# sarahappleby/VAMP

Measured on AMD Instinct MI355X. Metric: walker-steps/sec (log-posterior evals/sec), higher is better.
Workload: dtype f64

## Files before the change

### vamp_amd/csrc/vamp_hip.hip

```cpp
#include <hip/hip_runtime.h>
#include <dlfcn.h>

#include <algorithm>
#include <atomic>
#include <chrono>
#include <cmath>
#include <cstdint>
#include <cstdio>
#include <cstdlib>
#include <cstring>
#include <new>
#include <string>
#include <vector>

#include "../../include/vamp_hip.h"
#include "abi_state.hpp"
#include "draws.hpp"
#include "host_plan.hpp"
#include "map_search.hpp"
#include "voigt_math.hpp"
#include "ff_predicates.hpp"
#include "ff_moments.hpp"

#ifndef VAMP_EARLY_LOADS
#define VAMP_EARLY_LOADS 1
#endif
#ifndef VAMP_BLEND_PASS_LINES
#define VAMP_BLEND_PASS_LINES 4
#endif
#ifndef VAMP_MID_MIN_K
#define VAMP_MID_MIN_K 3
#endif
#ifndef VAMP_MID_MIN_P
#define VAMP_MID_MIN_P 96
#endif
#ifndef VAMP_X_PREFETCH
#define VAMP_X_PREFETCH 0
#endif

#ifndef VAMP_MIN_WAVES
#define VAMP_MIN_WAVES 3
#endif
#ifndef VAMP_EARLY_LNP
#define VAMP_EARLY_LNP 1
#endif
#ifndef VAMP_SR_EARLY
#define VAMP_SR_EARLY 0
#endif
#ifndef VAMP_XCD_MAP
#define VAMP_XCD_MAP 0
#endif
#ifndef VAMP_WIDE_NODES
#define VAMP_WIDE_NODES 1
#endif
#ifndef VAMP_LPT
#define VAMP_LPT 1
#endif
#ifndef VAMP_FLUX_EXP_DROP
#define VAMP_FLUX_EXP_DROP 2
#endif
#ifndef VAMP_FF_R2_M4
#define VAMP_FF_R2_M4 100.0
#define VAMP_FF_R2_M3 300.0
#define VAMP_FF_R2_M2 2000.0
#endif
#ifndef VAMP_F32_FAR_CORE
#define VAMP_F32_FAR_CORE 1
#endif
#ifndef VAMP_CORE_FASTPATH
#define VAMP_CORE_FASTPATH 1
#endif
#ifndef VAMP_MID_NODES
#define VAMP_MID_NODES 1
#endif
#ifndef VAMP_MID_Z2
#define VAMP_MID_Z2 30.25
#endif
#ifndef VAMP_WIDE_MAX
#define VAMP_WIDE_MAX 0.75
#endif
#ifndef VAMP_F32_LEAN_STAGE
#define VAMP_F32_LEAN_STAGE 1
#endif
#ifndef VAMP_TILE_MOMENTS
#define VAMP_TILE_MOMENTS 2
#endif
#ifndef VAMP_NODE_PASS
#define VAMP_NODE_PASS 1
#endif
#ifndef VAMP_NP_CLASS_RUNS
#define VAMP_NP_CLASS_RUNS 1
#endif
#ifndef VAMP_DEAL_ADJ
#define VAMP_DEAL_ADJ 1
#endif
#ifndef VAMP_SUPER_NODES
#define VAMP_SUPER_NODES 0
#endif
#ifndef VAMP_TAB_PAIR
#define VAMP_TAB_PAIR 0
#endif
#ifndef VAMP_TILE_HEAD
#define VAMP_TILE_HEAD 0
#endif
namespace {

constexpr int KMAX = 16;
constexpr int KMAX_ALL = VAMP_MAX_COMPONENTS;
static_assert(KMAX_ALL >= KMAX && KMAX_ALL < 64, "lane k stages line k; one spare lane for sd");
constexpr int WAVES_PER_BLOCK = 4;
constexpr long long PACK_MIN_WALKERS = 16384;
constexpr int RES_MAX_MOVERS = 128;
#ifndef VAMP_RES_WAVES
#define VAMP_RES_WAVES 8
#endif
constexpr int RES_MAX_WAVES = VAMP_RES_WAVES;
constexpr int BLOCK = 64 * WAVES_PER_BLOCK;
constexpr int DMAX = 4 * KMAX_ALL + 1;
#ifndef VAMP_SPLIT_MAX_WALKERS
#define VAMP_SPLIT_MAX_WALKERS (1ll << 62)
#endif
constexpr long long SPLIT_MAX_WALKERS = VAMP_SPLIT_MAX_WALKERS;

constexpr double C_LIGHT = 2.98e8;
constexpr double SIGMA0 = 0.0263;
constexpr double SQRT_LN2 = 0.83255461115769775635;
constexpr double SQRT_PI = 1.77245385090551602730;
constexpr double FWHM_PER_SIGMA = 2.35482004503094938202;
constexpr double NEG_INF = -__builtin_huge_val();

using vamp::RegionDev;

struct LineRec {
    double c;
    double s;
    double y;
    double amp;
    double pole;
    double hy;
    double xcap;
    double w8, w25;
    double wmid;
};

#ifndef VAMP_PARTS
#define VAMP_PARTS 4
#endif
constexpr int PARTS = VAMP_PARTS;
template <int KCAP, bool OWN_DTAB> struct WalkerLds;
#ifdef VAMP_STAMPS
__device__ unsigned long long g_stamps[2 * 8192];
__device__ unsigned int g_stamp_n;
#define VAMP_STAMP(tag)                                                                          \
    do {                                                                                         \
        if (blockIdx.x == 0 && threadIdx.x == 0) {                                               \
            const unsigned int n_ = g_stamp_n;                                                   \
            if (n_ < 8192) { g_stamps[2 * n_] = (tag); g_stamps[2 * n_ + 1] = __builtin_amdgcn_s_memtime(); g_stamp_n = n_ + 1; } \
        }                                                                                        \
    } while (0)
#define VAMP_STAMP_AFTER(tag, v) do { asm volatile("" :: "v"(v)); VAMP_STAMP(tag); } while (0)
#else
#define VAMP_STAMP(tag) do {} while (0)
#define VAMP_STAMP_AFTER(tag, v) do {} while (0)
#endif
#ifndef VAMP_SPLIT_WAVES
#define VAMP_SPLIT_WAVES 4
#endif
#ifndef VAMP_SPLIT_WAVES_F32
#define VAMP_SPLIT_WAVES_F32 4
#endif
#ifndef VAMP_F32_TABLES
#define VAMP_F32_TABLES 1
#endif
template <int LPW_, int KCAP_, bool TAIL_, int WPB_, bool SPLIT_ = false, bool TABS_ = SPLIT_, bool FF_ = (LPW_ == 64)>
struct Pack {
    static constexpr int LPW = LPW_, KCAP = KCAP_, SUBS = 64 / LPW_;
    static constexpr bool TAIL = TAIL_;
    static constexpr bool SPLIT = SPLIT_;
    static constexpr bool TABS = TABS_;
    static constexpr bool FF = FF_;
// ... 833 lines not shown
            const LineRec ln = L.line[k];
            double X[T], H[T];
#pragma unroll
            for (int t = 0; t < T; ++t) X[t] = fabs(xi[t] - ln.c) * ln.s;
            if (TAB && (((unsigned)zonemasks >> k) & 1u)) {
                table_eval_tile<T>(tab + k * vamp::TAB_LINE, X, H);
            } else {
                tile_voigt<T, TAB>(ln, dtab_row<PK>(L, k), X, H, TAB ? tab + k * vamp::TAB_LINE : nullptr, dct + FF_EXP);
            }
#pragma unroll
            for (int t = 0; t < T; ++t) tau[t] = fma(ln.amp, H[t], tau[t]);
        }
#endif
        double fi[T], wi[T];
        if (nfar + nwide > 0) {
            double u[T];
#pragma unroll
            for (int t = 0; t < T; ++t) u[t] = ut[base + 64 * t + lane];
#ifndef VAMP_SKIP_FFNODES
            double fs_wide = 0.0;
            if constexpr (WIDE) {
                if (nwide > 0) {
                    fs_wide = ff_wide_nodes<typename PK::Lds>(L, Sx.widelist[j], dct, tab, lane, nwide, mid, half);
                }
            }
            ff_coefficients<typename PK::Lds, GUARD>(L, Sx, Sx.farlist[j], dct, lane, nfar, mid, half, fs_wide);
#endif
#if VAMP_EARLY_LOADS
#pragma unroll
            for (int t = 0; t < T; ++t) {
                fi[t] = f[base + 64 * t + lane];
                wi[t] = wt[base + 64 * t + lane];
            }
            __builtin_amdgcn_sched_barrier(0);
#endif
#ifndef VAMP_SKIP_CLENSHAW
            ff_horner<double, T>(Sx, u, up, tau);
#endif
        } else {
#if VAMP_EARLY_LOADS
#pragma unroll
            for (int t = 0; t < T; ++t) {
                fi[t] = f[base + 64 * t + lane];
                wi[t] = wt[base + 64 * t + lane];
            }
            __builtin_amdgcn_sched_barrier(0);
#endif
        }
        int eoff = FF_EXP;
        asm volatile("" : "+s"(eoff));
        const double* ec = dct + eoff;
#pragma unroll
        for (int t = 0; t < T; ++t) {
#if !VAMP_EARLY_LOADS
            fi[t] = f[base + 64 * t + lane];
            wi[t] = wt[base + 64 * t + lane];
#endif
#ifdef VAMP_SKIP_EXP
            const double m = 1.0 - tau[t];
#else
            const double m = vamp::exp_taylor_tab<VAMP_FLUX_EXP_DROP>(-tau[t], ec);
#endif
            const double r = (fi[t] - m) * wi[t];
            chi = fma(r, r, chi);
        }
    }
    }
}

#if VAMP_NODE_PASS && VAMP_TILE_MOMENTS != 1 && !VAMP_X_PREFETCH && !defined(VAMP_SKIP_NEAR) && !defined(VAMP_SKIP_FFNODES) && \
    !defined(VAMP_SKIP_CLENSHAW) && !defined(VAMP_SKIP_EXP)
#define VAMP_NODE_PASS_ON 1
#else
#define VAMP_NODE_PASS_ON 0
#endif
#if VAMP_NODE_PASS_ON
__device__ __forceinline__ unsigned ff_fold16(unsigned long long m) {
    const unsigned h = (unsigned)m | (unsigned)(m >> 32);
    return (h | (h >> 16)) & 0xffffu;
}
#if VAMP_SUPER_NODES && VAMP_DEAL_ADJ
#define VAMP_SUPER_ON 1
#include "ff_super.inc"
struct NodeSets { unsigned far, n6, n4, n3, wide, dist, d3; double Mid, Half; };
#else
#define VAMP_SUPER_ON 0
struct NodeSets { unsigned far, n6, n4, n3, wide; };
#endif
template <bool WIDE, bool ZONE, class LDS>
__device__ __forceinline__ void ff_classify_batch_np(const LDS& L, const double2* __restrict__ geo, int K, int lane_, int base, int stride,
                                                     unsigned wide_all, unsigned long long& farmasks, unsigned long long& widemasks,
                                                     unsigned long long& zonemasks, NodeSets& sets, double& mid, double& half,
                                                     bool super_ok = false) {
    int lane = lane_;
    asm volatile("" : "+v"(lane));
    const int j = lane >> 4, k = lane & (KMAX - 1);
    const double2 g = geo[(base + j * stride) >> 8];
    mid = g.x, half = fabs(g.y);
    const LineRec& me = *reinterpret_cast<const LineRec*>(reinterpret_cast<const char*>(L.line) +
                                                          __umul24((unsigned)(k < K ? k : 0), (unsigned)sizeof(LineRec)));
    const double my_c = me.c, my_s = me.s, my_y = me.y, my_w8 = me.w8, my_wmid = me.wmid;
    const double dist = fabs(mid - my_c) - half;
    const bool my_beyond = (k < K) & (dist >= FF_DIST * half);
    const bool my_far = my_beyond & (dist >= my_w8);
    const double Xe = dist * my_s, r2e = fma(Xe, Xe, my_y * my_y);
    farmasks = __ballot(my_far);
    sets.far = ff_fold16(farmasks);
    sets.n6 = ff_fold16(__ballot(my_far & (r2e < VAMP_FF_R2_M4)));
    sets.n4 = ff_fold16(__ballot(my_far & (r2e < VAMP_FF_R2_M3)));
    sets.n3 = ff_fold16(__ballot(my_far & (r2e < VAMP_FF_R2_M2)));
    widemasks = 0ull;
    if constexpr (WIDE) {
        const bool my_wide = ((((wide_all >> k) & 1u) != 0u) | (VAMP_MID_NODES && (my_beyond & (dist >= my_wmid)))) & !my_far;
        widemasks = __ballot(my_wide);
    }
    sets.wide = ff_fold16(widemasks);
    zonemasks = 0ull;
    if constexpr (ZONE) zonemasks = __ballot(vamp::ff_tile_in_zone(my_c, my_s, my_y, mid, half));
#if VAMP_SUPER_ON
    sets.dist = sets.d3 = 0u;
    sets.Mid = sets.Half = 0.0;
    if (super_ok) {
        const double2 g0 = geo[base >> 8], g3 = geo[(base + (FF_BATCH - 1) * stride) >> 8];
        vamp::ff_super_tile(g0.x, fabs(g0.y), g3.x, fabs(g3.y), sets.Mid, sets.Half);
        const bool my_dist = (k < K) & vamp::ff_super_distant(my_c, my_s, my_y, sets.Mid, sets.Half);
        const bool my_d3 = my_dist & (vamp::ff_super_r2e(my_c, my_s, my_y, sets.Mid, sets.Half) < VAMP_FF_R2_M2);
        const unsigned all4 = (unsigned)farmasks & (unsigned)(farmasks >> 16) & (unsigned)(farmasks >> 32) & (unsigned)(farmasks >> 48) & 0xffffu;
        sets.dist = (unsigned)__ballot(my_dist) & all4;
        sets.d3 = (unsigned)__ballot(my_d3) & sets.dist;
        sets.far &= ~sets.dist, sets.n6 &= ~sets.dist, sets.n4 &= ~sets.dist, sets.n3 &= ~sets.dist;
    }
#endif
}
constexpr double FF_X_IDLE = 64.0;
static_assert(FF_X_IDLE * FF_X_IDLE >= VAMP_FF_R2_M2 && FF_X_IDLE < vamp::X_FAR, "the idle argument neither deepens a pair nor needs a guard");
template <int M> struct NpDepth { static constexpr int value = M; };
#if VAMP_SUPER_ON
template <class LDS>
__device__ __forceinline__ double ff_super_pass(const LDS& L, TileScratch& Sx, const double* __restrict__ dct, int lane, double xnode,
                                                const NodeSets& sets) {
    const vamp::SuperOrder ord = vamp::super_order(sets.dist, sets.d3);
    const int n = lane & (FF_NODES - 1), g4 = (lane >> 4) * 4;
    const double xs = fma(sets.Half, dct[FF_MAT + n], sets.Mid);
    unsigned long long seq = ord.seq;
    int left = ord.n;
    double acc = 0.0;
    auto run = [&](auto depth, int iters) {
        constexpr int M = decltype(depth)::value;
#pragma unroll 1
        for (int i = 0; i < iters; ++i) {
            const unsigned s32 = (unsigned)seq >> g4;
            double X[2], y[2], amp[2], r2[2], nn[2], d[2];
#pragma unroll
            for (int t = 0; t < 2; ++t) {
                const LineRec& ln = *reinterpret_cast<const LineRec*>(reinterpret_cast<const char*>(L.line) +
                                                                      __umul24((s32 >> (16 * t)) & 15u, (unsigned)sizeof(LineRec)));
                const bool live = (g4 >> 2) + 4 * t < left;
                const double Xl = fabs(xs - ln.c) * ln.s;
                X[t] = live ? Xl : FF_X_IDLE;
                y[t] = ln.y;
                amp[t] = live ? ln.amp : 0.0;
                r2[t] = fma(X[t], X[t], y[t] * y[t]);
                vamp::voigt_jfrac_nd<M>(X[t], y[t], r2[t], nn[t], d[t], vamp::GHFrac<M>::Z, vamp::GHFrac<M>::C);
            }
            const double ra = vamp::rcp_nr(d[0] * d[1]);
            acc = fma(amp[0], nn[0] * (ra * d[1]), acc);
            acc = fma(amp[1], nn[1] * (ra * d[0]), acc);
            seq >>= 32;
            left -= 8;
        }
    };
    run(NpDepth<3>{}, ord.iters3);
    run(NpDepth<2>{}, ord.iters - ord.iters3);
    {
        const int me = lane_here();
        const int a16 = (me ^ 16) << 2, a32 = (me ^ 32) << 2;
        acc += __hiloint2double(__builtin_amdgcn_ds_bpermute(a16, __double2hiint(acc)), __builtin_amdgcn_ds_bpermute(a16, __double2loint(acc)));
        acc += __hiloint2double(__builtin_amdgcn_ds_bpermute(a32, __double2hiint(acc)), __builtin_amdgcn_ds_bpermute(a32, __double2loint(acc)));
    }
    if (lane < FF_NODES) Sx.coef[lane] = acc;
    __builtin_amdgcn_wave_barrier();
    const double2* crow = reinterpret_cast<const double2*>(FF_SUPER_C) + n;
    const double2* fv = reinterpret_cast<const double2*>(Sx.coef);
    double a0 = 0.0, a1 = 0.0;
#pragma unroll
    for (int n2 = 0; n2 < FF_NODES / 2; ++n2) {
        const double2 m = crow[n2 * FF_NODES], f2 = fv[n2];
        a0 = fma(m.x, f2.x, a0);
        a1 = fma(m.y, f2.y, a1);
    }
    __builtin_amdgcn_wave_barrier();
    if (lane < FF_NODES) Sx.coef[lane] = a0 + a1;
    __builtin_amdgcn_wave_barrier();
    const double t = (xnode - sets.Mid) * vamp::rcp_nr(sets.Half), t2 = t + t;
    double b1 = 0.0, b2 = 0.0;
#pragma unroll
    for (int k = FF_NODES - 1; k >= 1; --k) {
        const double b = fma(t2, b1, Sx.coef[k] - b2);
        b2 = b1;
        b1 = b;
    }
    const double p = fma(t, b1, Sx.coef[0] - b2);
    __builtin_amdgcn_wave_barrier();
    return p;
}
#endif
template <bool WIDE, bool GUARD, class LDS>
__device__ __forceinline__ double ff_node_pass(const LDS& L, const double* __restrict__ dct, const double* tab, int lane_, double mid, double half,
                                               unsigned long long farmasks, unsigned long long widemasks, NodeSets sets,
                                               TileScratch* Sx = nullptr) {
    int lane = lane_;
    asm volatile("" : "+v"(lane));
    const double xnode = fma(half, dct[FF_MAT + (lane & (FF_NODES - 1))], mid);
    double fs = 0.0;
#if VAMP_SUPER_ON
    if (sets.dist != 0u) {
        fs = ff_super_pass(L, *Sx, dct, lane, xnode, sets);
        farmasks &= ~(sets.dist * 0x0001000100010001ull);
    }
#endif
    const unsigned far16 = ff_tile_field(farmasks, lane);
#if VAMP_NP_CLASS_RUNS
    if (sets.far != 0u) {
    const vamp::NpOrder ord = vamp::np_pair_order(sets.far, sets.n6, sets.n4, sets.n3);
    unsigned long long seq = ord.seq;
    const unsigned far16b = far16 & ~ord.solo;
    struct Pair { double c[2], s[2], y[2], amp[2]; };
    auto read_pair = [&](unsigned long long q) {
        Pair p;
#pragma unroll
        for (int t = 0; t < 2; ++t) {
            const LineRec& ln = L.line[(unsigned)(q >> (4 * t)) & 15u];
            p.c[t] = ln.c, p.s[t] = ln.s, p.y[t] = ln.y, p.amp[t] = ln.amp;
        }
        return p;
    };
    Pair nxt = read_pair(seq);
    auto run = [&](auto depth, int npairs, const double* Zt, const double* Ct) {
        constexpr int M = decltype(depth)::value;
#pragma unroll 1
        for (int i = 0; i < npairs; ++i) {
            const Pair p = nxt;
            const unsigned k0 = (unsigned)seq & 15u, k1 = (unsigned)(seq >> 4) & 15u;
            seq >>= 8;
            nxt = read_pair(seq);
            const bool mine[2] = {((far16 >> k0) & 1u) != 0u, ((far16b >> k1) & 1u) != 0u};
            double X[2], amp[2], H[2];
#pragma unroll
            for (int t = 0; t < 2; ++t) {
                const double Xl = fabs(xnode - p.c[t]) * p.s[t];
                X[t] = mine[t] ? Xl : FF_X_IDLE;
                amp[t] = mine[t] ? p.amp[t] : 0.0;
            }
            if constexpr (GUARD) {
                ff_eval2<true>(X, p.y, H, dct + FF_EXP);
            } else {
                const double r2[2] = {fma(X[0], X[0], p.y[0] * p.y[0]), fma(X[1], X[1], p.y[1] * p.y[1])};
                double n[2], d[2];
#pragma unroll
                for (int t = 0; t < 2; ++t) vamp::voigt_jfrac_nd<M>(X[t], p.y[t], r2[t], n[t], d[t], Zt, Ct);
                const double ra = vamp::rcp_nr(d[0] * d[1]);
                H[0] = n[0] * (ra * d[1]);
                H[1] = n[1] * (ra * d[0]);
            }
            fs = fma(amp[0], H[0], fs);
            fs = fma(amp[1], H[1], fs);
        }
    };
    if constexpr (GUARD) {
        run(NpDepth<2>{}, ord.pairs[0] + ord.pairs[1] + ord.pairs[2] + ord.pairs[3], nullptr, nullptr);
    } else {
        const int z6 = vamp::opaque_zero();
        run(NpDepth<6>{}, ord.pairs[0], vamp::GHFrac<6>::Z + z6, vamp::GHFrac<6>::C + z6);
        const int z4 = vamp::opaque_zero();
        run(NpDepth<4>{}, ord.pairs[1], vamp::GHFrac<4>::Z + z4, vamp::GHFrac<4>::C + z4);
        run(NpDepth<3>{}, ord.pairs[2], vamp::GHFrac<3>::Z, vamp::GHFrac<3>::C);
        run(NpDepth<2>{}, ord.pairs[3], vamp::GHFrac<2>::Z, vamp::GHFrac<2>::C);
    }
    }
#else
    unsigned rest = sets.far, n6 = sets.n6, n4 = sets.n4, n3 = sets.n3;
    while (rest) {
        const int depth = n6 ? 6 : n4 ? 4 : n3 ? 3 : 2;
        int kk[2];
        bool live[2];
#pragma unroll
        for (int t = 0; t < 2; ++t) {
            live[t] = rest != 0u;
            if (live[t]) {
                kk[t] = __builtin_ctz(n6 ? n6 : n4 ? n4 : n3 ? n3 : rest);
                const unsigned keep = ~(1u << kk[t]);
                rest &= keep, n6 &= keep, n4 &= keep, n3 &= keep;
            } else {
                kk[t] = kk[0];
            }
        }
        double X[2], y[2], amp[2], H[2];
#pragma unroll
        for (int t = 0; t < 2; ++t) {
            const LineRec& ln = L.line[kk[t]];
            const bool mine = live[t] & (((far16 >> kk[t]) & 1u) != 0u);
            X[t] = mine ? fabs(xnode - ln.c) * ln.s : FF_X_IDLE;
            y[t] = ln.y;
            amp[t] = mine ? ln.amp : 0.0;
        }
        if constexpr (GUARD) {
            ff_eval2<true>(X, y, H, dct + FF_EXP);
        } else {
            const double r2[2] = {fma(X[0], X[0], y[0] * y[0]), fma(X[1], X[1], y[1] * y[1])};
            if (depth == 6) ff_frac2<6>(X, y, r2, H);
            else if (depth == 4) ff_frac2<4>(X, y, r2, H);
            else if (depth == 3) ff_frac2<3>(X, y, r2, H);
            else ff_frac2<2>(X, y, r2, H);
        }
        fs = fma(amp[0], H[0], fs);
        fs = fma(amp[1], H[1], fs);
    }
#endif
    if constexpr (WIDE) {
        const unsigned wide16 = ff_tile_field(widemasks, lane);
        for (unsigned w = sets.wide; w; w &= w - 1u) {
            const int k = __builtin_ctz(w);
            if ((wide16 >> k) & 1u) {
                const LineRec& ln = L.line[k];
                const double X = fabs(xnode - ln.c) * ln.s, r2 = fma(X, X, ln.y * ln.y);
                double H;
                if (r2 < vamp::R2_CORE) {
                    H = table_eval(tab + k * vamp::TAB_LINE, X);
                } else {
                    H = vamp::voigt_jfrac<6>(X, ln.y, r2);
                    if (ln.y < vamp::Y_TINY) H += vamp::SQRT_PI * vamp::exp_neg_sq_tab(X, dct + FF_EXP);
                }
                fs = fma(ln.amp, H, fs);
            }
        }
    }
    return fs;
}
template <class real>
__device__ __forceinline__ void ff_series_row(TileScratch& Sx, const double* __restrict__ dct, int lane, int j, double fs) {
    if ((lane >> 4) == j) Sx.coef[lane & (FF_NODES - 1)] = fs;
    __builtin_amdgcn_wave_barrier();
    const double2* mrow = reinterpret_cast<const double2*>(dct) + (lane < FF_ROWS ? lane : FF_ROWS - 1);
    const double2* fv = reinterpret_cast<const double2*>(Sx.coef);
    double a0 = 0.0, a1 = 0.0;
#pragma unroll
    for (int n2 = 0; n2 < FF_NODES / 2; ++n2) {
        const double2 m = mrow[n2 * FF_ROWS], f2 = fv[n2];
        a0 = fma(m.x, f2.x, a0);
        a1 = fma(m.y, f2.y, a1);
    }
    __builtin_amdgcn_wave_barrier();
    if (lane < FF_ROWS) reinterpret_cast<real*>(Sx.coef)[lane] = (real)(a0 + a1);
    __builtin_amdgcn_wave_barrier();
}
__device__ __forceinline__ void ff_moment_chi_nodes_row(TileScratch& Sx, const double* __restrict__ mt, int lane, int j, double a_row, double c0,
                                                        double& chi) {
    if ((lane >> 4) == j) Sx.coef[lane & (FF_NODES - 1)] = a_row;
    const int n = lane & (FF_NODES - 1), g4 = (lane >> 4) * 4;
    const double2* Qr = reinterpret_cast<const double2*>(mt + vamp::FFN_Q + n * FF_NODES + g4);
    const double2 q01 = Qr[0], q23 = Qr[1];
    const double Sv = mt[vamp::FFN_S + n];
    __builtin_amdgcn_wave_barrier();
    const double2* av = reinterpret_cast<const double2*>(Sx.coef + g4);
    const double2 a01 = av[0], a23 = av[1];
    const double a = Sx.coef[n];
    const double acc0 = fma(q01.x, a01.x, 0.5 * Sv), acc1 = q01.y * a01.y;
    const double term = a * (fma(q23.x, a23.x, acc0) + fma(q23.y, a23.y, acc1));
    chi += lane == 0 ? term + c0 : term;
    __builtin_amdgcn_wave_barrier();
}
template <int MODE, class PK, bool TAB, bool WIDE = false, bool GUARD = true, bool SUPER = false>
__device__ __forceinline__ void sweep_range_ff_np(const RegionDev& R, const typename PK::Lds& L, TileScratch& Sx, const double* __restrict__ dct,
                                                  const double* __restrict__ x, const double* __restrict__ f,
                                                  const double* __restrict__ wt, const double* __restrict__ ut,
                                                  const double2* __restrict__ geo, int lane, int base0, int base1, int stride,
                                                  double& chi, const double* tab, unsigned long long wide_all = 0ull,
                                                  const double* __restrict__ mom = nullptr) {
    constexpr int T = TPIX;
    static_assert(PK::LPW == 64 && PK::KCAP <= 16, "far-field tiles: one walker per wavefront, <= 16 lines");
    const int K = R.K;
    const int ntile = base0 < base1 ? (base1 - base0 + stride - 1) / stride : 0;
#if VAMP_DEAL_ADJ
    (void)ntile;
    const int tstride = 64 * T, bstep = FF_BATCH * stride;
    const int bfull = __builtin_amdgcn_readfirstlane((base1 / bstep) * bstep);
    const int bfirst = FF_BATCH * base0, brest = bfull + base0;
#else
    const int tstride = stride, bstep = FF_BATCH * stride;
    const int bfull = __builtin_amdgcn_readfirstlane(base0 + (ntile / FF_BATCH) * (FF_BATCH * stride));
    const int bfirst = base0, brest = bfull;
#endif
    for (int batch = __builtin_amdgcn_readfirstlane(bfirst); batch < bfull; batch += bstep) {
    unsigned long long farmasks, widemasks, zonemasks;
    double fsn;
    {
        NodeSets sets;
        double mid_j, half_j;
#if VAMP_SUPER_ON
        ff_classify_batch_np<WIDE, TAB>(L, geo, K, lane, batch, tstride, (unsigned)wide_all, farmasks, widemasks, zonemasks, sets, mid_j, half_j,
                                        SUPER);
        fsn = ff_node_pass<WIDE, GUARD>(L, dct, tab, lane, mid_j, half_j, farmasks, widemasks, sets, &Sx);
#else
        ff_classify_batch_np<WIDE, TAB>(L, geo, K, lane, batch, tstride, (unsigned)wide_all, farmasks, widemasks, zonemasks, sets, mid_j, half_j);
        fsn = ff_node_pass<WIDE, GUARD>(L, dct, tab, lane, mid_j, half_j, farmasks, widemasks, sets);
#endif
    }
#if VAMP_TILE_MOMENTS == 2
    {
        unsigned long long fm = farmasks, wm = widemasks;
        double a_row = 0.0, amax_row = 0.0;
        bool have_a = false;
#pragma unroll 1
        for (int j = 0; j < FF_BATCH; ++j, fm >>= KMAX, wm >>= KMAX) {
            const unsigned farmask = (unsigned)fm & 0xffffu, widemask = WIDE ? (unsigned)wm & 0xffffu : 0u;
            if ((~(farmask | widemask) & ((1u << K) - 1u)) != 0u) continue;
            const double* mt = mom + ((batch + j * tstride) >> 8) * MOM_TILE;
            const double root_c0 = mt[MOM_RC], root_q0 = mt[MOM_RQ];
            if (!vamp::ff_moments_try(root_c0, root_q0)) continue;
            if (!have_a) {
                int eoff = FF_EXP;
                asm volatile("" : "+s"(eoff));
                a_row = -vamp::expm1_taylor_tab(-fsn, dct + eoff);
                amax_row = row16_max(fabs(a_row));
                have_a = true;
            }
            const double amax = __hiloint2double(__builtin_amdgcn_readlane(__double2hiint(amax_row), KMAX * j),
                                                 __builtin_amdgcn_readlane(__double2loint(amax_row), KMAX * j));
            if (!vamp::ff_moments_ok(root_c0, root_q0, amax)) continue;
            ff_moment_chi_nodes_row(Sx, mt, lane_here(), j, a_row, mt[vamp::FFN_C0], chi);
            const unsigned long long field = 0xffffull << (KMAX * j);
            farmasks |= field;
            widemasks |= field;
        }
    }
#endif
#pragma unroll 1
    for (int j = 0; j < FF_BATCH; ++j, farmasks >>= KMAX, widemasks >>= KMAX, zonemasks >>= KMAX) {
        const int base = batch + j * tstride;
        double xi[T], tau[T];
#if VAMP_TILE_HEAD
        if ((unsigned)farmasks & (unsigned)widemasks & 0xffffu) continue;
#endif
#pragma unroll
        for (int t = 0; t < T; ++t) {
            xi[t] = x[base + 64 * t + lane];
            tau[t] = 0.0;
        }
#if !VAMP_TILE_HEAD
        if ((unsigned)farmasks & (unsigned)widemasks & 0xffffu) continue;
#endif
        const bool up = __double2hiint(geo[base >> 8].y) >= 0;
        const unsigned farmask = (unsigned)farmasks & 0xffffu;
        const unsigned widemask = WIDE ? (unsigned)widemasks & 0xffffu : 0u;
        for (unsigned near = ~(farmask | widemask) & ((1u << K) - 1u); near; near &= near - 1u) {
            const int k = __builtin_ctz(near);
            const LineRec ln = L.line[k];
            double X[T], H[T];
#pragma unroll
            for (int t = 0; t < T; ++t) X[t] = fabs(xi[t] - ln.c) * ln.s;
            if (TAB && (((unsigned)zonemasks >> k) & 1u)) {
                table_eval_tile<T>(tab + k * vamp::TAB_LINE, X, H);
            } else {
                tile_voigt<T, TAB>(ln, dtab_row<PK>(L, k), X, H, TAB ? tab + k * vamp::TAB_LINE : nullptr, dct + FF_EXP);
            }
#pragma unroll
            for (int t = 0; t < T; ++t) tau[t] = fma(ln.amp, H[t], tau[t]);
        }
        double fi[T], wi[T];
        if ((farmask | widemask) != 0u) {
            double u[T];
#pragma unroll
            for (int t = 0; t < T; ++t) u[t] = ut[base + 64 * t + lane];
            ff_series_row<double>(Sx, dct, lane, j, fsn);
#if VAMP_EARLY_LOADS
#pragma unroll
            for (int t = 0; t < T; ++t) {
                fi[t] = f[base + 64 * t + lane];
                wi[t] = wt[base + 64 * t + lane];
            }
            __builtin_amdgcn_sched_barrier(0);
#endif
            ff_horner<double, T>(Sx, u, up, tau);
        } else {
#if VAMP_EARLY_LOADS
#pragma unroll
            for (int t = 0; t < T; ++t) {
// ... 344 lines not shown
        const double cw = wave_sum<64>(w2d * d), qw = wave_sum<64>(w2);
        if ((p & 63) == 0) {
            part[p >> 6][0] = qw;
            part[p >> 6][1] = cw;
        }
        __syncthreads();
        if (p == 0) {
            const double q0 = (part[0][0] + part[1][0]) + (part[2][0] + part[3][0]);
            const double C0 = (part[0][1] + part[1][1]) + (part[2][1] + part[3][1]);
            mt[vamp::FFN_C0] = C0;
            mt[vamp::FFN_RC] = sqrt(C0);
            mt[vamp::FFN_RQ] = sqrt(q0);
        }
        if (p > vamp::FFN_RQ - vamp::FFN_S && p < vamp::FFN_TILE - vamp::FFN_S) mt[vamp::FFN_S + p] = 0.0;
    }
#elif VAMP_TILE_MOMENTS
    if constexpr (!F32) {
        __shared__ double part[TPIX][2];
        double* mt = mom + (g0 >> 8) * vamp::FFM_TILE;
        const int lane = (int)threadIdx.x & 63;
        const double w2 = wt[g] * wt[g], d = f[g] - 1.0, w2d = w2 * d;
        double pw = 1.0;
        for (int n = 0; n < vamp::FFM_NQ; ++n) {
            const double sq = wave_sum<64>(w2 * pw);
            if (lane == 0) mt[q * vamp::FFM_QROW + n] = sq;
            if (n == 0 && lane == 0) part[q][0] = sq;
            if (n < vamp::FFM_NS) {
                const double ss = wave_sum<64>(w2d * pw);
                if (lane == 0) mt[vamp::FFM_S + q * vamp::FFM_NS + n] = ss;
            }
            pw *= ug;
        }
        const double c0 = wave_sum<64>(w2d * d);
        if (lane == 0) part[q][1] = c0;
        __syncthreads();
        if (threadIdx.x == 0) {
            const double q0 = (part[0][0] + part[1][0]) + (part[2][0] + part[3][0]);
            const double C0 = (part[0][1] + part[1][1]) + (part[2][1] + part[3][1]);
            mt[vamp::FFM_C0] = C0;
            mt[vamp::FFM_RC] = sqrt(C0);
            mt[vamp::FFM_RQ] = sqrt(q0);
            mt[3 * vamp::FFM_QROW + vamp::FFM_NQ] = 0.0;
        }
    }
#endif
}

template <bool F32, int MODE, class PK, bool TAB = use_tables<F32, MODE, PK>()>
__device__ __forceinline__ void sweep_class(const RegionDev& R, const typename PK::Lds& L, TileScratch& Sx, const double* __restrict__ dct,
                                            const PixPtrs& px, int lane, int base0, int full, int stride, bool tail, double& chi,
                                            const double* tab) {
    constexpr int TPIX = pixels_per_lane<PK>();
    if constexpr (F32) {
        const float* x = px.xf + R.pix_off; const float* f = px.ff + R.pix_off; const float* wt = px.wtf + R.pix_off;
        if constexpr (VAMP_FARFIELD && PK::FF && MODE != VAMP_GAUSS3 && TPIX == 4)
            sweep_range_f32_ff<MODE, PK, use_tables32<F32, MODE, PK>()>(R, L, Sx, dct, x, f, wt, px.uf + R.pix_off, px.geo + (R.pix_off >> 8),
                                                                        lane, base0, full, stride, chi, reinterpret_cast<const float*>(tab));
        else if (TPIX > 1) sweep_range_f32<MODE, PK, TPIX>(R, L, x, f, wt, lane, base0, full, stride, chi);
        if constexpr (PK::TAIL || TPIX == 1)
            if (tail) {
                const int from = TPIX > 1 ? full : 0;
                if constexpr (!PK::FF && TPIX > 1) {
                    const int nt = (R.P - from + PK::LPW - 1) / PK::LPW;
                    if constexpr (TPIX >= 4) { if (nt == 4) sweep_range_f32<MODE, PK, 4>(R, L, x, f, wt, lane, from, from + 1, 1 << 28, chi); }
                    if constexpr (TPIX >= 3) { if (nt == 3) sweep_range_f32<MODE, PK, 3>(R, L, x, f, wt, lane, from, from + 1, 1 << 28, chi); }
                    if (nt == 2) sweep_range_f32<MODE, PK, 2>(R, L, x, f, wt, lane, from, from + 1, 1 << 28, chi);
                    else if (nt == 1) sweep_range_f32<MODE, PK, 1>(R, L, x, f, wt, lane, from, from + 1, 1 << 28, chi);
                } else {
                    sweep_range_f32<MODE, PK, 1>(R, L, x, f, wt, lane, from, R.P, PK::LPW, chi);
                }
            }
    } else {
        const double* x = px.x + R.pix_off; const double* f = px.f + R.pix_off; const double* wt = px.wt + R.pix_off;
        if constexpr (VAMP_FARFIELD && PK::FF && MODE != VAMP_GAUSS3 && TPIX == 4) {
            const double* ut = px.u + R.pix_off;
            const double2* geo = px.geo + (R.pix_off >> 8);
            const double* mom = VAMP_TILE_MOMENTS ? px.mom + (R.pix_off >> 8) * MOM_TILE : nullptr;
            const int flags = __builtin_amdgcn_readfirstlane((int)(__double_as_longlong(L.theta[4 * PK::KCAP + 2]) & 0x3ffff));
            const bool guard = (flags >> 16) != 0;
            if constexpr (VAMP_WIDE_NODES && TAB) {
                const unsigned long long wide_all = (unsigned long long)(flags & 0xffff);
                if (VAMP_MID_NODES || wide_all) {
                    if (guard) sweep_range_ff_any<MODE, PK, TAB, true, true>(R, L, Sx, dct, x, f, wt, ut, geo, lane, base0, full, stride, chi, tab, wide_all, mom);
                    else if (VAMP_SUPER_ON && wide_all == 0ull)
                        sweep_range_ff_any<MODE, PK, TAB, true, false, true>(R, L, Sx, dct, x, f, wt, ut, geo, lane, base0, full, stride, chi, tab, wide_all, mom);
                    else sweep_range_ff_any<MODE, PK, TAB, true, false>(R, L, Sx, dct, x, f, wt, ut, geo, lane, base0, full, stride, chi, tab, wide_all, mom);
                } else {
                    if (guard) sweep_range_ff_any<MODE, PK, TAB, false, true>(R, L, Sx, dct, x, f, wt, ut, geo, lane, base0, full, stride, chi, tab, 0ull, mom);
                    else sweep_range_ff_any<MODE, PK, TAB, false, false, true>(R, L, Sx, dct, x, f, wt, ut, geo, lane, base0, full, stride, chi, tab, 0ull, mom);
                }
            } else {
                if (guard) sweep_range_ff_any<MODE, PK, TAB, false, true>(R, L, Sx, dct, x, f, wt, ut, geo, lane, base0, full, stride, chi, tab, 0ull, mom);
                else sweep_range_ff_any<MODE, PK, TAB, false, false, true>(R, L, Sx, dct, x, f, wt, ut, geo, lane, base0, full, stride, chi, tab, 0ull, mom);
            }
        } else if (TPIX > 1) sweep_range<MODE, PK, TPIX, TAB>(R, L, x, f, wt, lane, base0, full, stride, chi, tab);
        if constexpr (PK::TAIL || TPIX == 1)
            if (tail) {
                const int from = TPIX > 1 ? full : 0;
                if constexpr (!PK::FF && TPIX > 1) {
                    const int nt = (R.P - from + PK::LPW - 1) / PK::LPW;
                    if constexpr (TPIX >= 4) { if (nt == 4) sweep_range<MODE, PK, 4, TAB>(R, L, x, f, wt, lane, from, from + 1, 1 << 28, chi, tab); }
                    if constexpr (TPIX >= 3) { if (nt == 3) sweep_range<MODE, PK, 3, TAB>(R, L, x, f, wt, lane, from, from + 1, 1 << 28, chi, tab); }
                    if (nt == 2) sweep_range<MODE, PK, 2, TAB>(R, L, x, f, wt, lane, from, from + 1, 1 << 28, chi, tab);
                    else if (nt == 1) sweep_range<MODE, PK, 1, TAB>(R, L, x, f, wt, lane, from, from + 1, 1 << 28, chi, tab);
                } else {
                    sweep_range<MODE, PK, 1, TAB>(R, L, x, f, wt, lane, from, R.P, PK::LPW, chi, tab);
                }
            }
    }
}

template <int MODE, class PK, int T>
__device__ __forceinline__ void blend_chunk(const RegionDev& R, const typename PK::Lds& L, const double* __restrict__ x, int lane,
                                            int base, int k0, int kn, const double* tab, double (&tau)[4]) {
    double xi[T];
#pragma unroll
    for (int t = 0; t < T; ++t) {
        const int i = base + 64 * t + lane;
        xi[t] = x[i < R.P ? i : R.P - 1];
    }
    for (int kk = 0; kk < kn; ++kk) {
        const LineRec ln = L.line[k0 + kk];
        double X[T], H[T];
#pragma unroll
        for (int t = 0; t < T; ++t) X[t] = fabs(xi[t] - ln.c) * ln.s;
        tile_voigt<T, true>(ln, L.dtab[k0 + kk], X, H, tab + kk * vamp::TAB_LINE);
#pragma unroll
        for (int t = 0; t < T; ++t) tau[t] = fma(ln.amp, H[t], tau[t]);
    }
}
template <int MODE, class PK>
__device__ __forceinline__ void blend_chunk_n(const RegionDev& R, const typename PK::Lds& L, const double* __restrict__ x, int lane,
                                              int base, int tn, int k0, int kn, const double* tab, double (&tau)[4]) {
    if (tn >= 4) blend_chunk<MODE, PK, 4>(R, L, x, lane, base, k0, kn, tab, tau);
    else if (tn == 3) blend_chunk<MODE, PK, 3>(R, L, x, lane, base, k0, kn, tab, tau);
    else if (tn == 2) blend_chunk<MODE, PK, 2>(R, L, x, lane, base, k0, kn, tab, tau);
    else if (tn == 1) blend_chunk<MODE, PK, 1>(R, L, x, lane, base, k0, kn, tab, tau);
}
constexpr int BLEND_MAX_PIXELS = 512;
template <int MODE, class PK>
__device__ __forceinline__ double sweep_blend_passes(const RegionDev& R, const typename PK::Lds& L, const PixPtrs& px, int lane,
                                                     double* tab) {
    static_assert(PK::WPB == 1 && PK::LPW == 64, "one wavefront per walker");
    constexpr int LP = PK::LINES_PER_PASS;
    const double* __restrict__ x = px.x + R.pix_off;
    const double* __restrict__ f = px.f + R.pix_off;
    const double* __restrict__ wt = px.wt + R.pix_off;
    const int P = R.P, K = R.K;
    const int nt = (P + 63) >> 6;
    const int tn0 = nt < 4 ? nt : 4, tn1 = nt - tn0;
    double tau0[4] = {0.0, 0.0, 0.0, 0.0}, tau1[4] = {0.0, 0.0, 0.0, 0.0};
    for (int k0 = 0; k0 < K; k0 += LP) {
        const int kn = K - k0 < LP ? K - k0 : LP;
        for (int e = lane; e < kn * vamp::TAB_NI; e += 64) {
            const int kk = e / vamp::TAB_NI, i = e % vamp::TAB_NI, k = k0 + kk;
            vamp::taylor_table_row(i, L.line[k].y, L.dtab[k], L.line[k].pole, L.line[k].hy, tab + kk * vamp::TAB_LINE + i * vamp::TAB_NT);
        }
        group_barrier<PK>();
        blend_chunk_n<MODE, PK>(R, L, x, lane, 0, tn0, k0, kn, tab, tau0);
        if (tn1 > 0) blend_chunk_n<MODE, PK>(R, L, x, lane, 256, tn1, k0, kn, tab, tau1);
        group_barrier<PK>();
    }
    double chi = 0.0;
#pragma unroll
    for (int c = 0; c < 2; ++c) {
#pragma unroll
        for (int t = 0; t < 4; ++t) {
            const int i = 256 * c + 64 * t + lane;
            if (64 * (4 * c + t) < P) {
// ... 141 lines not shown
#endif
    VAMP_STAMP(4);
    if (chi_out) *chi_out = ssum;
    double v = lp + loglike_from_sum(R, L, ssum);
    if (v != v) v = NEG_INF;
    return v;
}

template <bool F32, int MODE, class PK>
__global__ __launch_bounds__(PK::THREADS, (min_waves<F32, PK>())) void k_lnprob(const RegionDev* __restrict__ regions, int region, PixPtrs px,
                                                  long long W, const double* __restrict__ theta,
                                                  double* __restrict__ lnprob, double* __restrict__ chi2,
                                                  const int* __restrict__ region_list) {
    const bool all = region < 0;
    if (all) region = region_list ? region_list[blockIdx.y] : (int)blockIdx.y;
    __shared__ typename PK::Lds lds[PK::SPLIT ? 1 : PK::WPB * PK::SUBS];
    __shared__ TileScratch scr[PK::FF ? PK::WPB : 1];
    __shared__ alignas(16) double dct[PK::FF ? ff_table_doubles<F32>() : 1];
    __shared__ double red[PARTS];
    __shared__ LineTables<table_doubles<F32, MODE, PK>()> tabs[PK::SPLIT ? 1 : PK::WPB];
    if constexpr (PK::FF) ff_fill_table<F32>(dct);
    const int wave = threadIdx.x >> 6, lane = threadIdx.x & 63;
    const int sub = lane / PK::LPW, l = lane % PK::LPW;
    const long long w = PK::SPLIT ? (long long)blockIdx.x : ((long long)blockIdx.x * PK::WPB + wave) * PK::SUBS + sub;
    if (w >= W) return;
    const RegionDev R = regions[region];
    if (all) {
        theta += W * R.d_before;
        lnprob += (long long)region * W;
        if (chi2) chi2 += (long long)region * W;
    }
    typename PK::Lds& L = lds[PK::SPLIT ? 0 : wave * PK::SUBS + sub];
    if (!PK::SPLIT || wave == 0)
        for (int d = l; d < R.D; d += PK::LPW) L.theta[d] = theta[w * R.D + d];
    group_barrier<PK>();
    double chi;
    const double v = wave_lnprob<F32, MODE, PK>(R, L, scr[PK::FF ? wave : 0], dct, px, l, &chi, wave, red,
                                                tabs[PK::SPLIT ? 0 : wave].a);
    if (PK::SPLIT && wave != 0) return;
    if (l == 0) {
        lnprob[w] = v;
        if (chi2) chi2[w] = chi;
    }
}

template <int MODE>
__global__ __launch_bounds__(PackSplit::THREADS) void k_dbg_node_sums(const RegionDev* __restrict__ regions, int region, PixPtrs px,
                                                                      const double* __restrict__ theta, double* __restrict__ nodes,
                                                                      unsigned* __restrict__ sets_out, bool adj_) {
    using PK = PackSplit;
    const bool adj = VAMP_DEAL_ADJ && adj_;
    __shared__ typename PK::Lds lds[1];
    __shared__ TileScratch scr[PK::WPB];
    __shared__ alignas(16) double dct[ff_table_doubles<false>()];
    __shared__ LineTables<table_doubles<false, MODE, PK>()> tabs[1];
    ff_fill_table<false>(dct);
    const int wave = threadIdx.x >> 6, lane = threadIdx.x & 63;
    const RegionDev R = regions[region];
    typename PK::Lds& L = lds[0];
    if (wave == 0)
        for (int d = lane; d < R.D; d += 64) L.theta[d] = theta[d];
    group_barrier<PK>();
    const double lp = stage_lines<MODE, PK, true, false, false, true>(R, L, lane, false, wave, tabs[0].a, px.x + R.pix_off);
    if (!(lp > NEG_INF)) return;
    TileScratch& Sx = scr[wave];
    const double* tab = tabs[0].a;
    const double2* geo = px.geo + (R.pix_off >> 8);
    const int flags = __builtin_amdgcn_readfirstlane((int)(__double_as_longlong(L.theta[4 * PK::KCAP + 2]) & 0x3ffff));
    const bool guard = (flags >> 16) != 0;
    const unsigned wide_all = (unsigned)(flags & 0xffff);
    constexpr int TILE = 64 * TPIX;
    const int K = R.K, base1 = (R.P / TILE) * TILE, stride = PARTS * TILE;
    const int base0 = __builtin_amdgcn_readfirstlane(wave * TILE);
    int bfull = base0, brest = base0;
#if VAMP_NODE_PASS_ON
    const int ntile = base0 < base1 ? (base1 - base0 + stride - 1) / stride : 0;
    const int tstride = adj ? TILE : stride, bstep = FF_BATCH * stride;
    bfull = __builtin_amdgcn_readfirstlane(adj ? (base1 / bstep) * bstep : base0 + (ntile / FF_BATCH) * bstep);
    brest = adj ? bfull + base0 : bfull;
    for (int batch = adj ? FF_BATCH * base0 : base0; batch < bfull; batch += bstep) {
        unsigned long long farmasks, widemasks, zonemasks;
        NodeSets sets;
        double mid, half;
        ff_classify_batch_np<true, true>(L, geo, K, lane, batch, tstride, wide_all, farmasks, widemasks, zonemasks, sets, mid, half,
                                         adj && !guard && wide_all == 0u);
        const double fs = guard ? ff_node_pass<true, true>(L, dct, tab, lane, mid, half, farmasks, widemasks, sets)
                                : ff_node_pass<true, false>(L, dct, tab, lane, mid, half, farmasks, widemasks, sets, &Sx);
        nodes[((batch + (lane >> 4) * tstride) >> 8) * FF_NODES + (lane & (FF_NODES - 1))] = fs;
        if (lane == 0) {
            unsigned* so = sets_out + (batch >> 8) * 5;
            so[0] = sets.far, so[1] = sets.n6, so[2] = sets.n4, so[3] = sets.n3, so[4] = sets.wide;
        }
    }
#endif
    for (int batch = brest; batch < base1; batch += FF_BATCH * stride) {
        unsigned long long farmasks, widemasks, zonemasks;
        ff_classify_batch<true, false, true>(L, Sx, geo, K, lane, batch, base1, stride, wide_all, farmasks, widemasks, zonemasks);
        for (int j = 0; j < FF_BATCH; ++j, farmasks >>= KMAX, widemasks >>= KMAX) {
            const int base = batch + j * stride;
            if (base >= base1) break;
            const double2 tg = geo[base >> 8];
            const double mid = tg.x, half = fabs(tg.y);
            const int nfar = __builtin_popcount((unsigned)farmasks & 0xffffu), nwide = __builtin_popcount((unsigned)widemasks & 0xffffu);
            const double fs_wide = nwide > 0 ? ff_wide_nodes<typename PK::Lds>(L, Sx.widelist[j], dct, tab, lane, nwide, mid, half) : 0.0;
            const double fs = guard ? ff_node_sums<typename PK::Lds, true>(L, Sx.farlist[j], dct, lane, nfar, mid, half, fs_wide)
                                    : ff_node_sums<typename PK::Lds, false>(L, Sx.farlist[j], dct, lane, nfar, mid, half, fs_wide);
            if (lane < FF_NODES) nodes[(base >> 8) * FF_NODES + lane] = fs;
        }
        __builtin_amdgcn_wave_barrier();
    }
}

constexpr int NM_INIT = 0, NM_CAND = 1, NM_CAND2 = 2, NM_SHRINK = 3;
constexpr int NM_LDS_DOUBLES = 34 * 33 + 2;
struct MapLds {
    double xbar[DMAX], worst[DMAX];
    double f[DMAX + 1];
    int ord[DMAX + 1];
    double fv[16];
    double redx[WAVES_PER_BLOCK], redf[WAVES_PER_BLOCK];
    double f0;
};
template <bool F32, int MODE, class PK>
__global__ __launch_bounds__(PK::THREADS, (min_waves<F32, PK>())) void k_map_search(
    const RegionDev* __restrict__ regions, PixPtrs px, const int* __restrict__ region_list, const double* __restrict__ theta0,
    const unsigned char* __restrict__ active, long long maxiter, long long maxfun, double xtol, double ftol,
    double* __restrict__ scratch, double* __restrict__ theta_best, long long* __restrict__ iterations) {
    constexpr int SLOTS = PK::WALKERS_PER_BLOCK, NT = PK::THREADS;
    static_assert(SLOTS <= 16 && PK::WPB <= WAVES_PER_BLOCK, "MapLds::fv / redx");
    __shared__ typename PK::Lds lds[PK::SPLIT ? 1 : PK::WPB * PK::SUBS];
    __shared__ TileScratch scr[PK::FF ? PK::WPB : 1];
    __shared__ alignas(16) double dct[PK::FF ? ff_table_doubles<F32>() : 1];
    __shared__ double red[PARTS];
    __shared__ LineTables<table_doubles<F32, MODE, PK>()> tabs[PK::SPLIT ? 1 : PK::WPB];
    __shared__ MapLds M;
    if constexpr (PK::FF) ff_fill_table<F32>(dct);
    const int tid = threadIdx.x;
    const int wave = tid >> 6, lane = tid & 63;
    const int sub = lane / PK::LPW, l = lane % PK::LPW;
    const int slot = PK::SPLIT ? 0 : wave * PK::SUBS + sub;
    const int region = region_list ? region_list[blockIdx.x] : (int)blockIdx.x;
    const RegionDev R = regions[region];
    const int N = R.D;
    theta0 += R.d_before;
    theta_best += R.d_before;
    if (active && !active[region]) {
        for (int d = tid; d < N; d += NT) theta_best[d] = theta0[d];
        if (tid == 0) iterations[region] = 0;
        return;
    }
    __shared__ double sim_lds[NM_LDS_DOUBLES];
    double* sim = (N + 1) * N <= NM_LDS_DOUBLES ? sim_lds : scratch + R.sim_off;
    typename PK::Lds& L = lds[slot];
    for (int e = tid; e < (N + 1) * N; e += NT) {
        const int k = e / N, d = e - k * N;
        const double v = theta0[d];
        sim[e] = (k >= 1 && d == k - 1) ? vamp::nm_start_coordinate(v) : v;
    }
    for (int k = tid; k <= N; k += NT) M.ord[k] = k;
    const long long fun_cap = maxfun > 0 ? maxfun : 200ll * N;
    int phase = NM_INIT, base = 0, need = 0;
    long long it = 0, calls = 0;
    for (;;) {
        __syncthreads();
        int n_pts = 0;
        if (phase == NM_CAND) {
            if (calls >= fun_cap || it + 1 >= maxiter) break;
            double mx = 0.0, mf = 0.0;
            for (int d = tid; d < N; d += NT) {
                const double r0 = sim[(long long)M.ord[0] * N + d];
// ... 1852 lines not shown
```

Before: 14.59 million.

## Enable super-node far-field pass and split it out of batch classification

Turns on the super-node path by default. It moves the super-tile distant-line classification and pass into a separate ff_super_batch helper that returns early when no line is distant, and keeps NodeSets small. It also sends the non-guard wide case through the SUPER template variant. The aim is to evaluate distant lines once per four-tile super tile through a Chebyshev series instead of per tile, while keeping register pressure low in the common path. The cost is extra ballots and geometry loads per batch, plus a risk of accuracy or divergence differences.

After: 15.20 million (median of 6 runs). 1.04x the previous value.

```diff
diff --git a/vamp_amd/csrc/vamp_hip.hip b/vamp_amd/csrc/vamp_hip.hip
--- a/vamp_amd/csrc/vamp_hip.hip
+++ b/vamp_amd/csrc/vamp_hip.hip
@@ -95,7 +95,7 @@
 #define VAMP_DEAL_ADJ 1
 #endif
 #ifndef VAMP_SUPER_NODES
-#define VAMP_SUPER_NODES 0
+#define VAMP_SUPER_NODES 1
 #endif
 #ifndef VAMP_TAB_PAIR
 #define VAMP_TAB_PAIR 0
@@ -1095,16 +1095,14 @@
 #if VAMP_SUPER_NODES && VAMP_DEAL_ADJ
 #define VAMP_SUPER_ON 1
 #include "ff_super.inc"
-struct NodeSets { unsigned far, n6, n4, n3, wide, dist, d3; double Mid, Half; };
 #else
 #define VAMP_SUPER_ON 0
+#endif
 struct NodeSets { unsigned far, n6, n4, n3, wide; };
-#endif
 template <bool WIDE, bool ZONE, class LDS>
 __device__ __forceinline__ void ff_classify_batch_np(const LDS& L, const double2* __restrict__ geo, int K, int lane_, int base, int stride,
                                                      unsigned wide_all, unsigned long long& farmasks, unsigned long long& widemasks,
-                                                     unsigned long long& zonemasks, NodeSets& sets, double& mid, double& half,
-                                                     bool super_ok = false) {
+                                                     unsigned long long& zonemasks, NodeSets& sets, double& mid, double& half) {
     int lane = lane_;
     asm volatile("" : "+v"(lane));
     const int j = lane >> 4, k = lane & (KMAX - 1);
@@ -1130,20 +1128,6 @@
     sets.wide = ff_fold16(widemasks);
     zonemasks = 0ull;
     if constexpr (ZONE) zonemasks = __ballot(vamp::ff_tile_in_zone(my_c, my_s, my_y, mid, half));
-#if VAMP_SUPER_ON
-    sets.dist = sets.d3 = 0u;
-    sets.Mid = sets.Half = 0.0;
-    if (super_ok) {
-        const double2 g0 = geo[base >> 8], g3 = geo[(base + (FF_BATCH - 1) * stride) >> 8];
-        vamp::ff_super_tile(g0.x, fabs(g0.y), g3.x, fabs(g3.y), sets.Mid, sets.Half);
-        const bool my_dist = (k < K) & vamp::ff_super_distant(my_c, my_s, my_y, sets.Mid, sets.Half);
-        const bool my_d3 = my_dist & (vamp::ff_super_r2e(my_c, my_s, my_y, sets.Mid, sets.Half) < VAMP_FF_R2_M2);
-        const unsigned all4 = (unsigned)farmasks & (unsigned)(farmasks >> 16) & (unsigned)(farmasks >> 32) & (unsigned)(farmasks >> 48) & 0xffffu;
-        sets.dist = (unsigned)__ballot(my_dist) & all4;
-        sets.d3 = (unsigned)__ballot(my_d3) & sets.dist;
-        sets.far &= ~sets.dist, sets.n6 &= ~sets.dist, sets.n4 &= ~sets.dist, sets.n3 &= ~sets.dist;
-    }
-#endif
 }
 constexpr double FF_X_IDLE = 64.0;
 static_assert(FF_X_IDLE * FF_X_IDLE >= VAMP_FF_R2_M2 && FF_X_IDLE < vamp::X_FAR, "the idle argument neither deepens a pair nor needs a guard");
@@ -1151,10 +1135,10 @@
 #if VAMP_SUPER_ON
 template <class LDS>
 __device__ __forceinline__ double ff_super_pass(const LDS& L, TileScratch& Sx, const double* __restrict__ dct, int lane, double xnode,
-                                                const NodeSets& sets) {
-    const vamp::SuperOrder ord = vamp::super_order(sets.dist, sets.d3);
+                                                unsigned dist, unsigned d3, double Mid, double Half) {
+    const vamp::SuperOrder ord = vamp::super_order(dist, d3);
     const int n = lane & (FF_NODES - 1), g4 = (lane >> 4) * 4;
-    const double xs = fma(sets.Half, dct[FF_MAT + n], sets.Mid);
+    const double xs = fma(Half, dct[FF_MAT + n], Mid);
     unsigned long long seq = ord.seq;
     int left = ord.n;
     double acc = 0.0;
@@ -1205,7 +1189,7 @@
     __builtin_amdgcn_wave_barrier();
     if (lane < FF_NODES) Sx.coef[lane] = a0 + a1;
     __builtin_amdgcn_wave_barrier();
-    const double t = (xnode - sets.Mid) * vamp::rcp_nr(sets.Half), t2 = t + t;
+    const double t = (xnode - Mid) * vamp::rcp_nr(Half), t2 = t + t;
     double b1 = 0.0, b2 = 0.0;
 #pragma unroll
     for (int k = FF_NODES - 1; k >= 1; --k) {
@@ -1217,21 +1201,37 @@
     __builtin_amdgcn_wave_barrier();
     return p;
 }
+template <class LDS>
+__device__ __forceinline__ double ff_super_batch(const LDS& L, TileScratch& Sx, const double* __restrict__ dct, const double2* __restrict__ geo,
+                                                 int K, int lane_, int base, int stride, double mid, double half,
+                                                 unsigned long long farmasks, NodeSets& sets) {
+    int lane = lane_;
+    asm volatile("" : "+v"(lane));
+    const int k = lane & (KMAX - 1);
+    const LineRec& me = *reinterpret_cast<const LineRec*>(reinterpret_cast<const char*>(L.line) +
+                                                          __umul24((unsigned)(k < K ? k : 0), (unsigned)sizeof(LineRec)));
+    const double my_c = me.c, my_s = me.s, my_y = me.y;
+    const double2 g0 = geo[base >> 8], g3 = geo[(base + (FF_BATCH - 1) * stride) >> 8];
+    double Mid, Half;
+    vamp::ff_super_tile(g0.x, fabs(g0.y), g3.x, fabs(g3.y), Mid, Half);
+    const bool my_dist = (k < K) & vamp::ff_super_distant(my_c, my_s, my_y, Mid, Half);
+    const bool my_d3 = my_dist & (vamp::ff_super_r2e(my_c, my_s, my_y, Mid, Half) < VAMP_FF_R2_M2);
+    const unsigned all4 = (unsigned)farmasks & (unsigned)(farmasks >> 16) & (unsigned)(farmasks >> 32) & (unsigned)(farmasks >> 48) & 0xffffu;
+    const unsigned dist = (unsigned)__ballot(my_dist) & all4;
+    if (dist == 0u) return 0.0;
+    const unsigned d3 = (unsigned)__ballot(my_d3) & dist;
+    sets.far &= ~dist, sets.n6 &= ~dist, sets.n4 &= ~dist, sets.n3 &= ~dist;
+    const double xnode = fma(half, dct[FF_MAT + (lane & (FF_NODES - 1))], mid);
+    return ff_super_pass(L, Sx, dct, lane, xnode, dist, d3, Mid, Half);
+}
 #endif
 template <bool WIDE, bool GUARD, class LDS>
 __device__ __forceinline__ double ff_node_pass(const LDS& L, const double* __restrict__ dct, const double* tab, int lane_, double mid, double half,
-                                               unsigned long long farmasks, unsigned long long widemasks, NodeSets sets,
-                                               TileScratch* Sx = nullptr) {
+                                               unsigned long long farmasks, unsigned long long widemasks, NodeSets sets, double fs0 = 0.0) {
     int lane = lane_;
     asm volatile("" : "+v"(lane));
     const double xnode = fma(half, dct[FF_MAT + (lane & (FF_NODES - 1))], mid);
-    double fs = 0.0;
-#if VAMP_SUPER_ON
-    if (sets.dist != 0u) {
-        fs = ff_super_pass(L, *Sx, dct, lane, xnode, sets);
-        farmasks &= ~(sets.dist * 0x0001000100010001ull);
-    }
-#endif
+    double fs = fs0;
     const unsigned far16 = ff_tile_field(farmasks, lane);
 #if VAMP_NP_CLASS_RUNS
     if (sets.far != 0u) {
@@ -1352,6 +1352,9 @@
 }
 template <class real>
 __device__ __forceinline__ void ff_series_row(TileScratch& Sx, const double* __restrict__ dct, int lane, int j, double fs) {
+#if VAMP_SUPER_ON
+    asm volatile("" : "+v"(lane));
+#endif
     if ((lane >> 4) == j) Sx.coef[lane & (FF_NODES - 1)] = fs;
     __builtin_amdgcn_wave_barrier();
     const double2* mrow = reinterpret_cast<const double2*>(dct) + (lane < FF_ROWS ? lane : FF_ROWS - 1);
@@ -1410,12 +1413,16 @@
     {
         NodeSets sets;
         double mid_j, half_j;
+        ff_classify_batch_np<WIDE, TAB>(L, geo, K, lane, batch, tstride, (unsigned)wide_all, farmasks, widemasks, zonemasks, sets, mid_j, half_j);
 #if VAMP_SUPER_ON
-        ff_classify_batch_np<WIDE, TAB>(L, geo, K, lane, batch, tstride, (unsigned)wide_all, farmasks, widemasks, zonemasks, sets, mid_j, half_j,
-                                        SUPER);
-        fsn = ff_node_pass<WIDE, GUARD>(L, dct, tab, lane, mid_j, half_j, farmasks, widemasks, sets, &Sx);
+        double fs0 = 0.0;
+        if constexpr (SUPER) {
+            if (__builtin_amdgcn_readfirstlane((int)(unsigned)wide_all) == 0) {
+                fs0 = ff_super_batch(L, Sx, dct, geo, K, lane, batch, tstride, mid_j, half_j, farmasks, sets);
+            }
+        }
+        fsn = ff_node_pass<WIDE, GUARD>(L, dct, tab, lane, mid_j, half_j, farmasks, widemasks, sets, fs0);
 #else
-        ff_classify_batch_np<WIDE, TAB>(L, geo, K, lane, batch, tstride, (unsigned)wide_all, farmasks, widemasks, zonemasks, sets, mid_j, half_j);
         fsn = ff_node_pass<WIDE, GUARD>(L, dct, tab, lane, mid_j, half_j, farmasks, widemasks, sets);
 #endif
     }
@@ -1926,9 +1933,7 @@
                 const unsigned long long wide_all = (unsigned long long)(flags & 0xffff);
                 if (VAMP_MID_NODES || wide_all) {
                     if (guard) sweep_range_ff_any<MODE, PK, TAB, true, true>(R, L, Sx, dct, x, f, wt, ut, geo, lane, base0, full, stride, chi, tab, wide_all, mom);
-                    else if (VAMP_SUPER_ON && wide_all == 0ull)
-                        sweep_range_ff_any<MODE, PK, TAB, true, false, true>(R, L, Sx, dct, x, f, wt, ut, geo, lane, base0, full, stride, chi, tab, wide_all, mom);
-                    else sweep_range_ff_any<MODE, PK, TAB, true, false>(R, L, Sx, dct, x, f, wt, ut, geo, lane, base0, full, stride, chi, tab, wide_all, mom);
+                    else sweep_range_ff_any<MODE, PK, TAB, true, false, true>(R, L, Sx, dct, x, f, wt, ut, geo, lane, base0, full, stride, chi, tab, wide_all, mom);
                 } else {
                     if (guard) sweep_range_ff_any<MODE, PK, TAB, false, true>(R, L, Sx, dct, x, f, wt, ut, geo, lane, base0, full, stride, chi, tab, 0ull, mom);
                     else sweep_range_ff_any<MODE, PK, TAB, false, false, true>(R, L, Sx, dct, x, f, wt, ut, geo, lane, base0, full, stride, chi, tab, 0ull, mom);
@@ -2236,10 +2241,13 @@
         unsigned long long farmasks, widemasks, zonemasks;
         NodeSets sets;
         double mid, half;
-        ff_classify_batch_np<true, true>(L, geo, K, lane, batch, tstride, wide_all, farmasks, widemasks, zonemasks, sets, mid, half,
-                                         adj && !guard && wide_all == 0u);
+        ff_classify_batch_np<true, true>(L, geo, K, lane, batch, tstride, wide_all, farmasks, widemasks, zonemasks, sets, mid, half);
+        double fs0 = 0.0;
+#if VAMP_SUPER_ON
+        if (adj && !guard && wide_all == 0u) fs0 = ff_super_batch(L, Sx, dct, geo, K, lane, batch, tstride, mid, half, farmasks, sets);
+#endif
         const double fs = guard ? ff_node_pass<true, true>(L, dct, tab, lane, mid, half, farmasks, widemasks, sets)
-                                : ff_node_pass<true, false>(L, dct, tab, lane, mid, half, farmasks, widemasks, sets, &Sx);
+                                : ff_node_pass<true, false>(L, dct, tab, lane, mid, half, farmasks, widemasks, sets, fs0);
         nodes[((batch + (lane >> 4) * tstride) >> 8) * FF_NODES + (lane & (FF_NODES - 1))] = fs;
         if (lane == 0) {
             unsigned* so = sets_out + (batch >> 8) * 5;
```
